# mbhall88/nohuman

Hardware: NVIDIA B200
Metric: classified+filtered throughput (Gbp/s) (higher is better)
Workload: dtype u64

## Files before the change

nohuman_b200/csrc/nh_kernels.cu:

```cuda
#include <stdlib.h>
#include <string.h>

#include "nh_kernels.cuh"

#define FULL_MASK 0xFFFFFFFFu


__device__ __forceinline__ uint32_t lane_id() { return threadIdx.x & 31u; }

__device__ __forceinline__ uint32_t warp_sum_u32(uint32_t v) {
  return __reduce_add_sync(FULL_MASK, v);
}

__device__ __forceinline__ uint64_t block_excl_scan(uint64_t v, uint64_t *total,
                                                    uint64_t *s_warp ) {
  uint32_t lane = lane_id(), warp = threadIdx.x >> 5;
  uint64_t inc = v;
#pragma unroll
  for (int d = 1; d < 32; d <<= 1) {
    uint64_t o = __shfl_up_sync(FULL_MASK, inc, d);
    if (lane >= (uint32_t)d) inc += o;
  }
  if (lane == 31) s_warp[warp] = inc;
  __syncthreads();
// ... 672 lines not shown
template <bool SMEM_PARENT>
__global__ void __launch_bounds__(NH_BLOCK_THREADS)
k_score(const NhDbParams db, const NhBatchPtrs b, const NhScoreParams sp) {
  extern __shared__ uint32_t s_dyn[];
  uint32_t *s_parent = s_dyn;
  const uint32_t parent_words = SMEM_PARENT ? db.node_count : 0u;
  uint32_t *s_hash = s_dyn + parent_words;
  if (SMEM_PARENT) {
    for (uint32_t i = threadIdx.x; i < db.node_count; i += blockDim.x) s_parent[i] = db.parent[i];
    __syncthreads();
  }
  const uint32_t *parent = SMEM_PARENT ? s_parent : db.parent;
  const uint32_t lane = lane_id(), warp = threadIdx.x >> 5;
  uint32_t *keys = s_hash + warp * 2u * NH_WARP_HASH_SLOTS;
  uint32_t *cnts = keys + NH_WARP_HASH_SLOTS;
  uint32_t classified = 0, kept = 0;
  const uint32_t wstride = gridDim.x * NH_WARPS_PER_BLOCK;
  const uint32_t n_todo = b.deferred_units ? b.counters->n_deferred : b.n_units;
  for (uint32_t i = blockIdx.x * NH_WARPS_PER_BLOCK + warp; i < n_todo; i += wstride) {
    const uint32_t u = b.deferred_units ? b.deferred_units[i] : i;
    acc_begin(keys, cnts, NH_WARP_HASH_SLOTS - 1u, lane);
    const UnitAcc a = b.tile_tab != nullptr ? acc_from_tile_tables(db, b, keys, cnts, NH_WARP_HASH_SLOTS - 1u, u, lane)
                                            : acc_from_lookups(db, b, keys, cnts, NH_WARP_HASH_SLOTS - 1u, u, lane);
    if (!resolve_unit(db, b, sp, parent, keys, cnts, NH_WARP_HASH_SLOTS - 1u, u, lane, a, &classified, &kept)) {
      if (lane == 0) b.overflow_units[atomicAdd(&b.counters->n_overflow, 1u)] = u;
    }
  }
  if (lane == 0) {
    if (classified) atomicAdd(&b.counters->n_classified, classified);
    if (kept) atomicAdd(&b.counters->n_kept, kept);
  }
}

__global__ void __launch_bounds__(32)
k_score_big(const NhDbParams db, const NhBatchPtrs b, const NhScoreParams sp) {
  extern __shared__ uint32_t s_dyn[];
  __shared__ MinWarpSmem s_min;
  uint32_t *keys = s_dyn;
  uint32_t *cnts = s_dyn + NH_BIG_HASH_SLOTS;
  const uint32_t lane = lane_id();
  const uint32_t n = b.counters->n_overflow;
  uint32_t classified = 0, kept = 0;
  for (uint32_t i = blockIdx.x; i < n; i += gridDim.x) {
    const uint32_t u = b.overflow_units[i];
    acc_begin(keys, cnts, NH_BIG_HASH_SLOTS - 1u, lane);
    const UnitAcc a = acc_rescan(db, b, keys, cnts, NH_BIG_HASH_SLOTS - 1u, u, lane, s_min);
    if (!resolve_unit(db, b, sp, db.parent, keys, cnts, NH_BIG_HASH_SLOTS - 1u, u, lane, a, &classified, &kept)) {
      if (db.huge_slots == 0u) {
        if (lane == 0) atomicExch(&b.counters->error, 1u);
        continue;
      }
      uint32_t *gkeys = db.huge_table, *gcnts = db.huge_table + db.huge_slots, *lock = db.huge_table + 2u * db.huge_slots;
      if (lane == 0)
        while (atomicCAS(lock, 0u, 1u) != 0u) __nanosleep(200);
      __syncwarp();
      __threadfence();
      acc_begin(gkeys, gcnts, db.huge_slots - 1u, lane);
      const UnitAcc ga = acc_rescan(db, b, gkeys, gcnts, db.huge_slots - 1u, u, lane, s_min);
      const bool ok = resolve_unit(db, b, sp, db.parent, gkeys, gcnts, db.huge_slots - 1u, u, lane, ga, &classified, &kept);
      __threadfence();
      __syncwarp();
      if (lane == 0) {
        atomicExch(lock, 0u);
        if (!ok) atomicExch(&b.counters->error, 1u);
      }
    }
  }
  if (lane == 0) {
    if (classified) atomicAdd(&b.counters->n_classified, classified);
    if (kept) atomicAdd(&b.counters->n_kept, kept);
  }
}


#ifndef NH_BCHUNK_WORDS
#define NH_BCHUNK_WORDS 8u
#endif
#define NH_BCHUNK_STRIDE (NH_BCHUNK_WORDS * 4u + 16u)
#ifndef NH_PQ_SLOTS
#define NH_PQ_SLOTS 128u
#endif
#define NH_META_FIRST 0x8000u
#define NH_AUX_NONE 0xFFFFFFFFu
#ifndef NH_FILTER_RECENT
#define NH_FILTER_RECENT 4u
#endif
#define NH_AUX_FILTER 0x80000000u

template <bool EMIT>
struct __align__(16) StreamWarpSmem {
  uint4 pq[NH_PQ_SLOTS];
  uint32_t q_unit[32];
  uint32_t q_ckey[32];
  uint32_t q_aux[32];
  uint64_t first_min[32], last_min[32];
  uint32_t keys[NH_LANE_TAXA * 32];
  uint32_t cnts[NH_LANE_TAXA * 32];
  uint32_t groups[32];
  uint8_t owner[32];
  uint32_t overflow;
  uint32_t first_hit;
  uint64_t bbar[2], sbar;
  __align__(16) uint8_t bchunk[2][32 * NH_BCHUNK_STRIDE];
  __align__(16) uint32_t sect[32 * 8];
  uint32_t q_slot[EMIT ? 32 : 1];
  uint8_t recent[32];
};

#ifndef NH_STREAM_MIN_BLOCKS
#define NH_STREAM_MIN_BLOCKS 3
#endif
static_assert((sizeof(StreamWarpSmem<false>) * NH_WARPS_PER_BLOCK + 1024 + 512) * NH_STREAM_MIN_BLOCKS <= 227 * 1024,
              "k_stream_classify would no longer fit its blocks per SM");

template <typename SM>
__device__ __forceinline__ uint32_t lane_tab_get(const SM &sm, uint32_t lane, uint32_t n, uint32_t taxon) {
  for (uint32_t i = 0; i < n; i++)
    if (sm.keys[i * 32u + lane] == taxon) return sm.cnts[i * 32u + lane];
  return 0;
}

__device__ __forceinline__ uint32_t smem_addr(const void *p) { return (uint32_t)__cvta_generic_to_shared(p); }
__device__ __forceinline__ void mbar_init(uint32_t bar, uint32_t count) {
  asm volatile("mbarrier.init.shared::cta.b64 [%0], %1;" ::"r"(bar), "r"(count) : "memory");
}
__device__ __forceinline__ void cp_async16(uint32_t dst, const void *src) {
  asm volatile("cp.async.cg.shared.global [%0], [%1], 16;" ::"r"(dst), "l"(src) : "memory");
}
__device__ __forceinline__ void cp_async8(uint32_t dst, const void *src) {
  asm volatile("cp.async.ca.shared.global [%0], [%1], 8;" ::"r"(dst), "l"(src) : "memory");
}
__device__ __forceinline__ void cp_async4(uint32_t dst, const void *src) {
  asm volatile("cp.async.ca.shared.global [%0], [%1], 4;" ::"r"(dst), "l"(src) : "memory");
}
__device__ __forceinline__ void cp_async16_zfill(uint32_t dst, const void *src, uint32_t n_src) {
  asm volatile("cp.async.cg.shared.global [%0], [%1], 16, %2;" ::"r"(dst), "l"(src), "r"(n_src) : "memory");
}
__device__ __forceinline__ void cp_async16_l2_64(uint32_t dst, const void *src) {
  asm volatile("cp.async.cg.shared.global.L2::64B [%0], [%1], 16;" ::"r"(dst), "l"(src) : "memory");
}
__device__ __forceinline__ void cp_async_arrive(uint32_t bar) {
  asm volatile("cp.async.mbarrier.arrive.noinc.shared::cta.b64 [%0];" ::"r"(bar) : "memory");
}
__device__ __forceinline__ void mbar_wait(uint32_t bar, uint32_t parity) {
  asm volatile(
      "{\n"
      ".reg .pred p;\n"
      "NH_WAIT:\n"
      "mbarrier.try_wait.parity.shared::cta.b64 p, [%0], %1;\n"
      "@p bra NH_DONE;\n"
      "bra NH_WAIT;\n"
      "NH_DONE:\n"
      "}" ::"r"(bar),
      "r"(parity)
      : "memory");
}
__device__ __forceinline__ uint32_t lds_u32(uint32_t addr) {
  uint32_t v;
  asm volatile("ld.shared.u32 %0, [%1];" : "=r"(v) : "r"(addr));
  return v;
}


__device__ __forceinline__ uint32_t nh_filter_hash(uint32_t ckey) {
  uint32_t h = ckey * 0x9E3779B1u;
  h ^= h >> 15;
  h *= 0x85EBCA77u;
  h ^= h >> 13;
  return h;
}

__global__ void __launch_bounds__(256)
k_filter_build(const uint32_t *__restrict__ cells, uint64_t capacity, uint32_t value_bits, uint32_t value_mask,
               uint32_t *__restrict__ filter, uint32_t n_blocks) {
  const uint32_t blk = blockIdx.x * blockDim.x + threadIdx.x;
  if (blk >= n_blocks) return;
  uint32_t rec[8];
#pragma unroll
  for (int i = 0; i < 8; i++) rec[i] = 0;
  const uint64_t base = (uint64_t)blk * 32ULL;
#pragma unroll 1
  for (uint32_t q = 0; q < 8; q++) {
    uint32_t c[4] = {0u, 0u, 0u, 0u};
    if (base + q * 4u + 4u <= capacity) {
      const uint4 v = __ldg(reinterpret_cast<const uint4 *>(cells + base) + q);
      c[0] = v.x; c[1] = v.y; c[2] = v.z; c[3] = v.w;
    } else {
      for (uint32_t j = 0; j < 4; j++)
        if (base + q * 4u + j < capacity) c[j] = __ldg(cells + base + q * 4u + j);
    }
#pragma unroll
    for (uint32_t j = 0; j < 4; j++) {
      const uint32_t cell = q * 4u + j;
      if (base + cell >= capacity) {
        rec[0] |= 1u << cell;
      } else if (c[j] & value_mask) {
        rec[0] |= 1u << cell;
        const uint32_t h = nh_filter_hash(c[j] >> value_bits);
        const uint32_t i0 = h & 63u, i1 = (h >> 6) & 63u, i2 = (h >> 12) & 63u, i3 = (h >> 18) & 31u;
        rec[1 + (i0 >> 5)] |= 1u << (i0 & 31u);
        rec[3 + (i1 >> 5)] |= 1u << (i1 & 31u);
        rec[5 + (i2 >> 5)] |= 1u << (i2 & 31u);
        rec[7] |= 1u << i3;
      }
    }
  }
  uint4 *out = reinterpret_cast<uint4 *>(filter + (uint64_t)blk * 8ULL);
  out[0] = make_uint4(rec[0], rec[1], rec[2], rec[3]);
  out[1] = make_uint4(rec[4], rec[5], rec[6], rec[7]);
}

#ifndef NH_STREAM_CHECK_MASK
#define NH_STREAM_CHECK_MASK 1
#endif

template <int W, int KL, bool DBG, bool REV0, bool EMIT, bool PACKED, int FILTER>
__global__ void __launch_bounds__(NH_BLOCK_THREADS, NH_STREAM_MIN_BLOCKS)
k_stream_classify(const NhDbParams db, const NhBatchPtrs b, const NhScoreParams sp) {
  static_assert(W == 5, "the scan consumes one 4-byte word per ring rotation");
  static_assert(NH_PQ_SLOTS >= 31u + 32u * (NH_STREAM_CHECK_MASK + 1u), "runs closed between two probe checks must fit the ring");
  static_assert((NH_PQ_SLOTS & (NH_PQ_SLOTS - 1u)) == 0 && (NH_BCHUNK_WORDS & (NH_BCHUNK_WORDS - 1u)) == 0, "powers of two");
  typedef StreamWarpSmem<EMIT> Smem;
  extern __shared__ __align__(16) uint32_t s_dyn[];
  uint32_t *s_parent = s_dyn;
  const bool smem_parent = db.node_count <= NH_SMEM_PARENT_MAX;
  const uint32_t parent_words = smem_parent ? db.node_count : 0u;
  Smem *s_warps = reinterpret_cast<Smem *>(s_dyn + ((parent_words + 3u) & ~3u));
  if (smem_parent) {
    for (uint32_t i = threadIdx.x; i < db.node_count; i += blockDim.x) s_parent[i] = db.parent[i];
    __syncthreads();
  }
  const uint32_t *parent = smem_parent ? s_parent : db.parent;
  const uint32_t lane = lane_id(), warp = threadIdx.x >> 5;
  const uint32_t lane_lt = (1u << lane) - 1u;
  Smem &sm = s_warps[warp];
  const uint32_t n_tiles = b.counters->n_tiles;
  const int k = KL ? 35 : db.k, l = KL ? 31 : db.l;
  const uint32_t amb_span = KL ? 34u : (uint32_t)db.amb_span;
  const uint64_t lmask = (1ULL << (2 * l)) - 1ULL;
  const uint32_t rc_shift = 2u * (uint32_t)(l - 1);
  const uint32_t n_sectors = (uint32_t)((db.capacity + 7ULL) >> 3);
  const uint32_t last_sector = n_sectors - 1u;
  const uint32_t last_range = (db.capacity & 7ULL) ? (1u << (uint32_t)(db.capacity & 7ULL)) - 1u : 0xFFu;
  const uint32_t max_visits = FILTER ? (n_sectors + 1u < 0x7FFEu ? n_sectors + 1u : 0x7FFEu) : (n_sectors + 1u < 0xFFFFu ? n_sectors + 1u : 0xFFFFu);
  const uint32_t last_block = FILTER ? sp.n_filter_blocks - 1u : 0u;
  const uint32_t ck_bits = 32u - db.value_bits;
  uint32_t tot_lookups = 0, tot_sectors = 0, tot_classified = 0, tot_kept = 0;

  const uint32_t bar0 = smem_addr(&sm.bbar[0]);
  const uint32_t win0 = smem_addr(&sm.bchunk[0][lane * NH_BCHUNK_STRIDE]);
  const uint32_t sbar = smem_addr(&sm.sbar);
  const uint32_t sect0 = smem_addr(&sm.sect[0]);
  uint32_t bar_par = 0;
  uint32_t sect_par = 0;
  if (lane == 0) {
    mbar_init(bar0, 32u);
    mbar_init(bar0 + 8u, 32u);
    mbar_init(sbar, 32u);
    asm volatile("fence.mbarrier_init.release.cluster;" ::: "memory");
  }
  asm volatile("fence.proxy.async.shared::cta;" ::: "memory");
  __syncwarp();

  for (;;) {
    uint32_t group = 0;
    if (lane == 0) group = atomicAdd(&b.counters->next_group, 1u);
    group = __shfl_sync(FULL_MASK, group, 0);
    if ((uint64_t)group * 32ULL >= n_tiles) break;
    const uint32_t tile = group * 32u + lane;
    const bool have = tile < n_tiles;
    NhTile t;
    t.seq = 0; t.pos_begin = 0; t.slot = 0; t.role = NH_ROLE_DEFERRED;
    if (have) t = b.tiles[tile];
    const uint32_t kind = NH_ROLE_KIND(t.role);
    const uint32_t owner = kind == NH_ROLE_MEMBER ? lane - NH_ROLE_DELTA(t.role) : lane;
#pragma unroll
    for (int i = 0; i < NH_LANE_TAXA; i++) {
      sm.keys[i * 32 + lane] = 0;
      sm.cnts[i * 32 + lane] = 0;
    }
    sm.groups[lane] = 0;
    if (FILTER == 3) sm.recent[lane] = 0;
    sm.owner[lane] = (uint8_t)owner;
    if (lane == 0) {
      sm.overflow = 0;
      sm.first_hit = 0;
    }
    __syncwarp();

    uint32_t pq_head = 0, pq_n = 0, cq_n = 0;
    uint32_t n_popped = 0;
    uint32_t n_conts = 0;
    uint32_t f_unit = 0, f_ckey = 0, f_slot = 0, f_aux = NH_AUX_NONE, f_start = 0;
    bool any_inflight = false;

    auto probe_round = [&]() {
      if (any_inflight) {
        const bool active = f_aux != NH_AUX_NONE;
        bool done = false;
        uint32_t result = 0;
        mbar_wait(sbar, sect_par);
        sect_par ^= 1u;
        if (active) {
          uint32_t c[8];
          {
            const uint4 lo = *reinterpret_cast<const uint4 *>(&sm.sect[lane * 8u]);
            const uint4 hi = *reinterpret_cast<const uint4 *>(&sm.sect[lane * 8u + 4u]);
            c[0] = lo.x; c[1] = lo.y; c[2] = lo.z; c[3] = lo.w;
            c[4] = hi.x; c[5] = hi.y; c[6] = hi.z; c[7] = hi.w;
          }
          if (FILTER) {
            const uint32_t ck = f_ckey & ((1u << ck_bits) - 1u);
            const uint32_t st = f_ckey >> ck_bits;
            const uint32_t visits = ((f_aux >> 16) & 0x7FFFu) + 1u;
            f_ckey = ck;
            if (f_aux & NH_AUX_FILTER) {
              const uint32_t h = nh_filter_hash(ck);
              const uint32_t w0 = (h & 32u) ? c[2] : c[1], w1 = (h & (32u << 6)) ? c[4] : c[3], w2 = (h & (32u << 12)) ? c[6] : c[5];
              const bool maybe = (((w0 >> (h & 31u)) & (w1 >> ((h >> 6) & 31u)) & (w2 >> ((h >> 12) & 31u)) & (c[7] >> ((h >> 18) & 31u))) & 1u) != 0u;
              const uint32_t free_cells = ~c[0] & (0xFFFFFFFFu << st);
              if (!maybe && free_cells != 0u) {
                done = true;
              } else if (visits >= max_visits) {
                done = true;
                atomicOr(&sm.overflow, FULL_MASK);
              } else if (maybe) {
                f_aux = (f_aux & 0xFFFFu) | (visits << 16);
                f_unit = f_unit * 4u + (st >> 3);
                f_ckey = ck | ((st & 7u) << ck_bits);
              } else {
                f_aux = (f_aux & (NH_AUX_FILTER | 0xFFFFu)) | (visits << 16);
                f_unit = f_unit == last_block ? 0u : f_unit + 1u;
              }
            } else {
              uint32_t range = 0xFFu << st;
              if (f_unit == last_sector) range &= last_range;
              int state = -1;
#pragma unroll
              for (int j = 7; j >= 0; j--) {
                const uint32_t val = c[j] & db.value_mask;
                const bool term = (val == 0u) || ((c[j] >> db.value_bits) == ck);
                if (term && ((range >> j) & 1u)) state = (int)val;
              }
              if (state >= 0) {
                done = true;
                result = (uint32_t)state;
              } else if (visits >= max_visits) {
                done = true;
                atomicOr(&sm.overflow, FULL_MASK);
              } else {
                f_aux = (f_aux & 0xFFFFu) | (visits << 16);
                f_unit = f_unit == last_sector ? 0u : f_unit + 1u;
              }
            }
          } else {
          uint32_t range = 0xFFu << f_start;
          if (f_unit == last_sector) range &= last_range;
          int state = -1;
#pragma unroll
          for (int j = 7; j >= 0; j--) {
            const uint32_t val = c[j] & db.value_mask;
            const bool term = (val == 0u) || ((c[j] >> db.value_bits) == f_ckey);
            if (term && ((range >> j) & 1u)) state = (int)val;
          }
          if (state >= 0) {
            done = true;
            result = (uint32_t)state;
          } else {
            const uint32_t visits = (f_aux >> 16) + 1u;
            if (visits >= max_visits) {
              done = true;
              if (EMIT) result = cht_walk(db, (uint64_t)f_unit * 8ULL + f_start, f_ckey);
              else atomicOr(&sm.overflow, FULL_MASK);
            } else {
              f_aux = (f_aux & 0xFFFFu) | (visits << 16);
              f_unit = f_unit == last_sector ? 0u : f_unit + 1u;
            }
          }
          }
        }
        const bool cont = active && !done;
        const uint32_t cmask = __ballot_sync(FULL_MASK, cont);
        if (cont) {
          const uint32_t pos = cq_n + __popc(cmask & lane_lt);
          sm.q_unit[pos] = f_unit;
          sm.q_ckey[pos] = f_ckey;
          sm.q_aux[pos] = f_aux;
          if (EMIT) sm.q_slot[pos] = f_slot;
        }
        cq_n += __popc(cmask);
        if (active && done) {
          const uint32_t tile_lane = f_aux & 31u;
          if (EMIT) b.lk_taxon[f_slot] = result;
          if (FILTER == 3) {
            const uint32_t r = sm.recent[tile_lane];
            if (result) sm.recent[tile_lane] = NH_FILTER_RECENT;
            else if (r) sm.recent[tile_lane] = (uint8_t)(r - 1u);
          }
          if (result) {
            const uint32_t own = sm.owner[tile_lane];
            const uint32_t n = (f_aux >> 5) & 0x3FFu;
            if (f_aux & NH_META_FIRST) atomicOr(&sm.first_hit, 1u << tile_lane);
            atomicAdd(&sm.groups[own], 1u);
            int i = 0;
            for (; i < sp.lane_taxa; i++) {
              const uint32_t old = atomicCAS(&sm.keys[i * 32 + own], 0u, result);
              if (old == 0u || old == result) {
                atomicAdd(&sm.cnts[i * 32 + own], n);
                break;
              }
            }
            if (i == sp.lane_taxa) atomicOr(&sm.overflow, 1u << own);
          }
        }
      }
      __syncwarp();
      const uint32_t n_cq = cq_n;
      const uint32_t room = 32u - n_cq;
      const uint32_t n_pq = pq_n < room ? pq_n : room;
      f_aux = NH_AUX_NONE;
      f_start = 0;
      if (lane < n_cq) {
        f_unit = sm.q_unit[lane];
        f_ckey = sm.q_ckey[lane];
        f_aux = sm.q_aux[lane];
        if (EMIT) f_slot = sm.q_slot[lane];
      } else if (lane - n_cq < n_pq) {
        const uint4 e = sm.pq[(pq_head + (lane - n_cq)) & (NH_PQ_SLOTS - 1u)];
        const uint64_t h = nh_fmix64(((uint64_t)e.y << 32) | e.x);
        if (EMIT) f_slot = e.w;
        const uint32_t meta = e.z;
        if (db.min_hash && h < db.min_hash) {
          if (EMIT) b.lk_taxon[f_slot] = 0u;
        } else {
          const uint64_t idx = nh_fastmod(h, db.capacity, db.mod_m, db.mod_sh1, db.mod_sh2);
          if (FILTER) {
            const bool ask = FILTER == 2 || (FILTER == 3 ? sm.recent[meta & 31u] == 0u : sm.groups[sm.owner[meta & 31u]] == 0u);
            const uint32_t st = (uint32_t)idx & (ask ? 31u : 7u);
            f_unit = (uint32_t)(idx >> (ask ? 5 : 3));
            f_ckey = (uint32_t)(h >> (32u + db.value_bits)) | (st << ck_bits);
            f_aux = ask ? (meta | NH_AUX_FILTER) : meta;
          } else {
            f_unit = (uint32_t)(idx >> 3);
            f_start = (uint32_t)idx & 7u;
            f_ckey = (uint32_t)(h >> (32u + db.value_bits));
            f_aux = meta;
          }
        }
      }
      cq_n = 0;
      pq_head = (pq_head + n_pq) & (NH_PQ_SLOTS - 1u);
      pq_n -= n_pq;
      n_popped += n_pq;
      n_conts += n_cq;
      any_inflight = (n_cq + n_pq) != 0u;
      if (any_inflight) {
        const uint32_t mine = f_aux != NH_AUX_NONE ? f_unit : 0xFFFFFFFFu;
        const uint32_t half = lane & 1u, src_lane = lane >> 1;
        const uint32_t u0 = __shfl_sync(FULL_MASK, mine, src_lane);
        const uint32_t u1 = __shfl_sync(FULL_MASK, mine, 16u + src_lane);
        const uint32_t dst = sect0 + src_lane * 32u + half * 16u;
        const uint32_t *src0 = db.cells, *src1 = db.cells;
        if (FILTER) {
          const uint32_t fmask = __ballot_sync(FULL_MASK, f_aux != NH_AUX_NONE && (f_aux & NH_AUX_FILTER));
          if ((fmask >> src_lane) & 1u) src0 = sp.filter;
          if ((fmask >> (16u + src_lane)) & 1u) src1 = sp.filter;
        }
        if (u0 != 0xFFFFFFFFu) cp_async16_l2_64(dst, src0 + (uint64_t)u0 * 8ULL + half * 4u);
        if (u1 != 0xFFFFFFFFu) cp_async16_l2_64(dst + 512u, src1 + (uint64_t)u1 * 8ULL + half * 4u);
        cp_async_arrive(sbar);
      }
      __syncwarp();
    };

    uint32_t n_runs = 0;
    uint32_t first_flag = NH_META_FIRST;
    uint64_t last = NH_NONE64;
    {
      uint64_t so = 0;
      uint32_t nb = 0;
      if (have) {
        so = b.offsets[t.seq];
        const uint32_t len = (uint32_t)(b.offsets[t.seq + 1] - so);
        uint32_t npos = len - (uint32_t)k + 1u - t.pos_begin;
        if (npos > (uint32_t)db.tile_pos) npos = (uint32_t)db.tile_pos;
        nb = npos + (uint32_t)k - 1u;
      }
      const uint8_t *g = PACKED ? nullptr : b.bases + so + t.pos_begin;
      const uint32_t mis = PACKED ? 0u : (uint32_t)((uintptr_t)g & 3u);
      const uint32_t my_words = have ? (mis + nb + 3u) >> 2 : 0u;
      const uint32_t max_words = __reduce_max_sync(FULL_MASK, my_words);

      uint64_t fwd = 0, rc = 0;
      uint64_t ring[4], pair[2];
#pragma unroll
      for (int i = 0; i < 4; i++) ring[i] = NH_NONE64;
      pair[0] = pair[1] = NH_NONE64;
      uint32_t c_run = 0;
      uint32_t cnt = 0;
      const uint64_t dbg_base = DBG && have ? b.dbg_pos_offsets[t.seq] + t.pos_begin : 0;
      const uint32_t first_pos = mis + (uint32_t)(k - 1);
      const uint32_t end_idx = mis + nb;

      auto emit = [&](bool pred, uint64_t key, uint32_t count) {
        const uint32_t emask = __ballot_sync(FULL_MASK, pred);
        if (pred) {
          uint4 e;
          e.x = (uint32_t)key;
          e.y = (uint32_t)(key >> 32);
          e.z = lane | (count << 5) | first_flag;
          e.w = 0;
          if (EMIT) {
            e.w = t.slot + n_runs;
            b.lk_cnt[e.w] = (uint16_t)count;
          }
          sm.pq[(pq_head + pq_n + __popc(emask & lane_lt)) & (NH_PQ_SLOTS - 1u)] = e;
          if (first_flag) sm.first_min[lane] = key;
          first_flag = 0;
          if (EMIT || DBG) n_runs++;
        }
        pq_n += __popc(emask);
      };

      auto scan_quad = [&](const uint32_t codes , const uint32_t ambs, const uint32_t base_i) {
#pragma unroll
        for (int j = 0; j < 4; j++) {
          const uint32_t i = base_i + (uint32_t)j;
          const uint32_t cc = (codes >> (6u - 2u * (uint32_t)j)) & 3u;
          const bool amb = (ambs >> j) & 1u;
          fwd = ((fwd << 2) | cc) & lmask;
          rc = (rc >> 2) | ((uint64_t)(3u - cc) << rc_shift);
          c_run = amb ? 0u : c_run + 1u;
          uint64_t cand = NH_NONE64;
          if (c_run >= (uint32_t)l) {
            const bool rev0 = REV0 || (DBG && db.revcom_version == 0);
            const uint64_t rcv = rev0 ? (((rc << (64 - 2 * l)) | ((1ULL << (64 - 2 * l)) - 1ULL)) & lmask) : rc;
            cand = ((fwd < rcv ? fwd : rcv) & db.seed_mask) ^ db.toggle;
          }
          const uint64_t a_i = min_u64(cand, ring[0]);
          const uint64_t m = min_u64(min_u64(a_i, pair[1]), ring[3]);
          pair[1] = pair[0];
          pair[0] = a_i;
#pragma unroll
          for (int r = 3; r > 0; r--) ring[r] = ring[r - 1];
          ring[0] = cand;
          const bool nonamb = i >= first_pos && c_run >= amb_span;
          const uint64_t mz = m ^ db.toggle;
          if (DBG && i >= first_pos && i < end_idx) {
            const uint64_t o = dbg_base + (i - first_pos);
            b.dbg_pos_min[o] = mz;
            b.dbg_pos_ambig[o] = nonamb ? 0 : 1;
          }
          const bool newrun = nonamb && mz != last;
          emit(newrun && cnt != 0u, last, cnt);
          cnt = newrun ? 1u : cnt + (nonamb ? 1u : 0u);
          last = newrun ? mz : last;
          if ((j & NH_STREAM_CHECK_MASK) == NH_STREAM_CHECK_MASK) {
            while (pq_n >= 32u) probe_round();
          }
        }
      };

      auto scan_word = [&](const uint32_t word, const uint32_t base_i) {
        uint32_t ambs;
        const uint32_t codes = nh_pack4(word, &ambs);
        scan_quad(codes, ambs, base_i);
      };

      if (PACKED) {
        const uint64_t unit0 = have ? (uint64_t)b.poff[t.seq] + (t.pos_begin >> 5) : 0ULL;
        const uint32_t my_units = have ? (nb + 31u) >> 5 : 0u;
        const uint32_t n_chunks = (max_words + 7u) >> 3;
        auto stage = [&](const uint32_t ch) {
          const uint32_t buf = ch & 1u;
          const uint32_t dst = win0 + buf * (32u * NH_BCHUNK_STRIDE);
          if (ch < my_units) {
            cp_async8(dst, b.codes + (unit0 + ch) * 8ULL);
            cp_async4(dst + 8u, b.valid + unit0 + ch);
          }
          cp_async_arrive(bar0 + buf * 8u);
        };
        if (n_chunks) stage(0u);
        for (uint32_t ch = 0; ch < n_chunks; ch++) {
          if (ch + 1u < n_chunks) stage(ch + 1u);
          const uint32_t buf = ch & 1u;
          mbar_wait(bar0 + buf * 8u, (bar_par >> buf) & 1u);
          bar_par ^= 1u << buf;
          const uint32_t wbase = win0 + buf * (32u * NH_BCHUNK_STRIDE);
          const uint32_t c_lo = lds_u32(wbase), c_hi = lds_u32(wbase + 4u);
          uint32_t vw = lds_u32(wbase + 8u);
          const int rem = (int)nb - (int)(ch * 32u);
          vw = rem <= 0 ? 0u : (rem >= 32 ? vw : vw & ((1u << rem) - 1u));
          const uint32_t amb_w = ~vw;
          const uint32_t q0 = ch * 8u;
          const uint32_t qn = max_words - q0 < 8u ? max_words - q0 : 8u;
#pragma unroll 1
          for (uint32_t qd = 0; qd < qn; qd++) {
            const uint32_t cw = qd < 4u ? c_lo : c_hi;
            scan_quad((cw >> ((qd & 3u) * 8u)) & 0xFFu, (amb_w >> (qd * 4u)) & 0xFu, (q0 + qd) * 4u);
          }
          __syncwarp();
        }
        emit(cnt != 0u, last, cnt);
      } else {
      const uint8_t *q = g - mis;
      const uint32_t a16 = (uint32_t)((uintptr_t)q & 15u);
      const uint8_t *src0 = q - a16;
      const uint32_t my_bytes = have ? a16 + mis + nb : 0u;
      const uint32_t n_chunks = (max_words + NH_BCHUNK_WORDS - 1u) / NH_BCHUNK_WORDS;
      auto stage = [&](const uint32_t ch) {
        const uint32_t buf = ch & 1u;
        const uint32_t lo = ch * (NH_BCHUNK_WORDS * 4u);
        const uint32_t dst = win0 + buf * (32u * NH_BCHUNK_STRIDE);
#pragma unroll
        for (uint32_t pc = 0; pc < NH_BCHUNK_STRIDE; pc += 16u) {
          const uint32_t at = lo + pc;
          const uint32_t n_src = at < my_bytes ? (my_bytes - at < 16u ? my_bytes - at : 16u) : 0u;
          cp_async16_zfill(dst + pc, n_src ? src0 + at : src0, n_src);
        }
        cp_async_arrive(bar0 + buf * 8u);
      };
      if (n_chunks) stage(0u);
      for (uint32_t ch = 0; ch < n_chunks; ch++) {
        if (ch + 1u < n_chunks) stage(ch + 1u);
        const uint32_t buf = ch & 1u;
        mbar_wait(bar0 + buf * 8u, (bar_par >> buf) & 1u);
        bar_par ^= 1u << buf;
        const uint32_t wbase = win0 + buf * (32u * NH_BCHUNK_STRIDE) + a16;
        const uint32_t w0 = ch * NH_BCHUNK_WORDS;
        const uint32_t wn = max_words - w0 < NH_BCHUNK_WORDS ? max_words - w0 : NH_BCHUNK_WORDS;
        uint32_t w_next = lds_u32(wbase);
        if (ch == 0u) w_next &= 0xFFFFFFFFu << (8u * mis);
#pragma unroll 1
        for (uint32_t w = 0; w < wn; w++) {
          const uint32_t word = w_next;
          w_next = lds_u32(wbase + (((w + 1u) & (NH_BCHUNK_WORDS - 1u)) << 2));
          scan_word(word, (w0 + w) * 4u);
        }
        __syncwarp();
      }
      emit(cnt != 0u, last, cnt);
      }
    }
    const bool has_runs = first_flag == 0u;
    if (EMIT && have) {
      NhTileOut o;
      o.lk_off = t.slot;
      o.lk_cnt = n_runs;
      b.tile_out[tile] = o;
    }
    if (has_runs) sm.last_min[lane] = last;
    while (pq_n + cq_n != 0u || any_inflight) probe_round();
    tot_lookups += n_popped;
    tot_sectors += n_popped + n_conts;

    {
      __syncwarp();
      const uint32_t has_mask = __ballot_sync(FULL_MASK, has_runs);
      if (have && kind != NH_ROLE_DEFERRED && t.pos_begin != 0u && has_runs && ((sm.first_hit >> lane) & 1u)) {
        const uint32_t seq_lane = lane - t.pos_begin / (uint32_t)db.tile_pos;
        const uint32_t cand = has_mask & lane_lt & ~((1u << seq_lane) - 1u);
        if (cand) {
          const uint32_t pl = 31u - (uint32_t)__clz(cand);
          if (sm.last_min[pl] == sm.first_min[lane]) atomicSub(&sm.groups[owner], 1u);
        }
      }
      __syncwarp();
    }

    if (have && kind == NH_ROLE_DEFERRED) {
      const bool ovf = (sm.overflow >> lane) & 1u;
      NhTileSum ts;
      ts.first_min = has_runs ? sm.first_min[lane] : NH_NONE64;
      ts.last_min = has_runs ? last : NH_NONE64;
      ts.groups = sm.groups[lane];
      ts.flags = (has_runs ? NH_TILE_HAS : 0u) | (((sm.first_hit >> lane) & 1u) ? NH_TILE_FIRST_HIT : 0u) |
                 (ovf ? NH_TILE_OVERFLOW : 0u);
      b.tile_sum[tile] = ts;
      if (!ovf) {
        NhTileTab tt;
#pragma unroll
        for (int i = 0; i < NH_LANE_TAXA; i++) {
          tt.keys[i] = sm.keys[i * 32 + lane];
          tt.cnts[i] = sm.cnts[i * 32 + lane];
        }
        b.tile_tab[tile] = tt;
      }
    }

    if (have && kind == NH_ROLE_LEADER) {
      const uint32_t u = b.paired ? (t.seq >> 1) : t.seq;
      if ((sm.overflow >> lane) & 1u) {
        b.overflow_units[atomicAdd(&b.counters->n_overflow, 1u)] = u;
      } else {
        uint32_t ntab = 0;
        while (ntab < (uint32_t)sp.lane_taxa && sm.keys[ntab * 32u + lane] != 0u) ntab++;
        const int groups = (int)sm.groups[lane];
        const uint32_t total_kmers = unit_total_kmers(db, b, u);
        uint32_t best_s = 0, best_t = 0;
        for (uint32_t i = 0; i < ntab; i++) {
          const uint32_t tx = sm.keys[i * 32u + lane];
          uint32_t score = 0;
          for (uint32_t a = tx; a; a = parent[a]) score += lane_tab_get(sm, lane, ntab, a);
          if (score > best_s) {
            best_s = score;
            best_t = tx;
          } else if (score == best_s) {
            best_t = lca(parent, best_t, tx);
          }
        }
        uint32_t max_taxon = best_t;
        uint32_t max_score = max_taxon ? lane_tab_get(sm, lane, ntab, max_taxon) : 0u;
        const uint32_t required = (uint32_t)ceil(__dmul_rn(sp.confidence, (double)total_kmers));
        while (max_taxon && max_score < required) {
          uint32_t sum = 0;
          for (uint32_t i = 0; i < ntab; i++)
            if (is_a_ancestor_of_b(parent, max_taxon, sm.keys[i * 32u + lane]))
              sum += sm.cnts[i * 32u + lane];
          max_score = sum;
          if (max_score >= required) break;
          max_taxon = parent[max_taxon];
        }
        uint32_t call = max_taxon;
        if (call && groups < sp.min_hit_groups) call = 0;
        const uint32_t is_cls = call != 0u;
        const uint32_t keep = sp.keep_human ? is_cls : !is_cls;
        if (b.out_call) b.out_call[u] = call ? db.ext_id[call] : 0u;
        if (b.out_keep) b.out_keep[u] = (uint8_t)keep;
        if (b.dbg_call) b.dbg_call[u] = call;
        if (b.dbg_total_kmers) b.dbg_total_kmers[u] = total_kmers;
        if (b.dbg_hit_groups) b.dbg_hit_groups[u] = (uint32_t)groups;
        tot_classified += is_cls;
        tot_kept += keep;
      }
    }
    __syncwarp();
  }
  tot_classified = warp_sum_u32(tot_classified);
  tot_kept = warp_sum_u32(tot_kept);
  if (lane == 0) {
    if (tot_lookups) atomicAdd(&b.counters->n_lookups, tot_lookups);
    if (tot_sectors) atomicAdd(&b.counters->n_sector_reads, tot_sectors);
    if (tot_classified) atomicAdd(&b.counters->n_classified, tot_classified);
    if (tot_kept) atomicAdd(&b.counters->n_kept, tot_kept);
  }
}


__global__ void __launch_bounds__(NH_BLOCK_THREADS)
k_gather_runs(const NhDbParams db, const NhBatchPtrs b, uint32_t *__restrict__ run_ext,
              uint16_t *__restrict__ run_len, uint32_t *__restrict__ tile_run_off,
              uint32_t *__restrict__ cursor) {
  const uint32_t lane = lane_id(), warp = threadIdx.x >> 5;
  const uint32_t n_tiles = b.counters->n_tiles;
  for (uint32_t tile = blockIdx.x * NH_WARPS_PER_BLOCK + warp; tile < n_tiles;
       tile += gridDim.x * NH_WARPS_PER_BLOCK) {
    const NhTileOut to = b.tile_out[tile];
    uint32_t base = 0;
    if (lane == 0) base = to.lk_cnt ? atomicAdd(cursor, to.lk_cnt) : 0u;
    base = __shfl_sync(FULL_MASK, base, 0);
    if (lane == 0) tile_run_off[tile] = base;
    for (uint32_t j = lane; j < to.lk_cnt; j += 32u) {
      run_ext[base + j] = db.ext_id[b.lk_taxon[to.lk_off + j]];
      run_len[base + j] = b.lk_cnt[to.lk_off + j];
    }
  }
}

__device__ __forceinline__ void fetch_sector_async(const uint32_t *cells, uint64_t sector, uint32_t smem_slot0, uint32_t lane) {
  const uint32_t half = lane & 1u, src_lane = lane >> 1;
  const uint64_t u0 = __shfl_sync(FULL_MASK, sector, src_lane);
  const uint64_t u1 = __shfl_sync(FULL_MASK, sector, 16u + src_lane);
  const uint32_t dst = smem_slot0 + src_lane * 32u + half * 16u;
  cp_async16_l2_64(dst, cells + u0 * 8ULL + half * 4u);
  cp_async16_l2_64(dst + 512u, cells + u1 * 8ULL + half * 4u);
}

template <int DEPTH>
__global__ void __launch_bounds__(256)
k_probe_pattern_async(const uint32_t *__restrict__ cells, uint64_t n_sectors, uint32_t items_per_chain,
                      uint32_t p_thresh, uint64_t seed, unsigned long long *__restrict__ counters,
                      uint32_t *__restrict__ sink) {
  __shared__ __align__(16) uint32_t s_sect[8][DEPTH][32 * 8];
  const uint32_t lane = lane_id(), warp = threadIdx.x >> 5;
  const uint64_t chain0 = ((uint64_t)blockIdx.x * blockDim.x + threadIdx.x) * DEPTH;
  uint64_t blk[DEPTH];
  uint32_t left[DEPTH], cont[DEPTH];
  uint32_t acc = 0;
  unsigned long long items = 0, requests = 0;
#pragma unroll
  for (int d = 0; d < DEPTH; d++) {
    blk[d] = __umul64hi(nh_fmix64(seed + (chain0 + d) * 0x9E3779B97F4A7C15ULL), n_sectors);
    left[d] = items_per_chain;
    cont[d] = 0;
    fetch_sector_async(cells, blk[d], smem_addr(&s_sect[warp][d][0]), lane);
    asm volatile("cp.async.commit_group;" ::: "memory");
  }
  for (uint32_t it = 1; it <= 2u * items_per_chain + 2u; it++) {
#pragma unroll
    for (int d = 0; d < DEPTH; d++) {
      asm volatile("cp.async.wait_group %0;" ::"n"(DEPTH - 1) : "memory");
      __syncwarp();
      const uint4 lo = *reinterpret_cast<const uint4 *>(&s_sect[warp][d][lane * 8u]);
      const uint4 hi = *reinterpret_cast<const uint4 *>(&s_sect[warp][d][lane * 8u + 4u]);
      const uint32_t x = lo.x ^ lo.y ^ lo.z ^ lo.w ^ hi.x ^ hi.y ^ hi.z ^ hi.w;
      __syncwarp();
      if (left[d] != 0u) {
        acc ^= x;
        requests++;
        const uint64_t h = nh_fmix64(seed ^ ((chain0 + d) << 20) ^ it ^ (uint64_t)(x & 1u) << 63);
        if (!cont[d] && (uint32_t)h < p_thresh) {
          cont[d] = 1;
          blk[d] = blk[d] + 1 < n_sectors ? blk[d] + 1 : 0;
        } else {
          cont[d] = 0;
          items++;
          left[d]--;
          blk[d] = __umul64hi(h, n_sectors);
        }
      }
      fetch_sector_async(cells, blk[d], smem_addr(&s_sect[warp][d][0]), lane);
      asm volatile("cp.async.commit_group;" ::: "memory");
    }
    if (!__any_sync(FULL_MASK, left[0] != 0u || left[DEPTH - 1] != 0u)) break;
  }
  asm volatile("cp.async.wait_group 0;" ::: "memory");
  if (acc == 0x9E3779B9u) sink[0] = acc;
  items = __reduce_add_sync(FULL_MASK, (uint32_t)items);
  requests = __reduce_add_sync(FULL_MASK, (uint32_t)requests);
  if (lane == 0) {
    atomicAdd(&counters[0], items);
    atomicAdd(&counters[1], requests);
  }
}

template <int G, int DEPTH>
__global__ void __launch_bounds__(256)
k_probe_pattern(const uint32_t *__restrict__ cells, uint64_t n_sectors, uint32_t items_per_chain,
                uint32_t p_thresh , uint64_t seed, uint64_t sm_window_sectors,
                unsigned long long *__restrict__ counters , uint32_t *__restrict__ sink) {
  const uint32_t lane = lane_id();
  const uint32_t sub = lane % G;
  const uint64_t chain0 = (((uint64_t)blockIdx.x * blockDim.x + threadIdx.x) / G) * DEPTH;
  uint64_t win_base = 0, win_size = n_sectors / G;
  if (sm_window_sectors) {
    uint32_t smid;
    asm("mov.u32 %0, %%smid;" : "=r"(smid));
    win_size = sm_window_sectors / G;
    const uint64_t n_win = (n_sectors / G) / win_size;
    win_base = (uint64_t)(smid % (uint32_t)(n_win ? n_win : 1)) * win_size;
  }
  uint32_t acc = 0;
  uint32_t c[DEPTH][8];
  uint64_t blk[DEPTH];
  uint32_t left[DEPTH];
  uint32_t cont[DEPTH];
  unsigned long long items = 0, requests = 0;
#pragma unroll
  for (int d = 0; d < DEPTH; d++) {
    const uint64_t h = nh_fmix64(seed + (chain0 + d) * 0x9E3779B97F4A7C15ULL);
    blk[d] = win_base + __umul64hi(h, win_size);
    left[d] = items_per_chain;
    cont[d] = 0;
    ld_sector(cells + (blk[d] * G + sub) * 8ULL, c[d]);
  }
  bool busy = true;
  for (uint32_t it = 1; busy; it++) {
    busy = false;
#pragma unroll
    for (int d = 0; d < DEPTH; d++) {
      if (left[d] == 0u) continue;
      busy = true;
      const uint32_t x = c[d][0] ^ c[d][1] ^ c[d][2] ^ c[d][3] ^ c[d][4] ^ c[d][5] ^ c[d][6] ^ c[d][7];
      acc ^= x;
      requests++;
      const uint64_t h = nh_fmix64(seed ^ ((chain0 + d) << 20) ^ it ^ (uint64_t)(x & 1u) << 63);
      if (!cont[d] && (uint32_t)h < p_thresh) {
        cont[d] = 1;
        blk[d] = blk[d] + 1 < win_base + win_size ? blk[d] + 1 : win_base;
      } else {
        cont[d] = 0;
        items++;
        if (--left[d] == 0u) continue;
        blk[d] = win_base + __umul64hi(h, win_size);
      }
      ld_sector(cells + (blk[d] * G + sub) * 8ULL, c[d]);
    }
  }
  if (acc == 0x9E3779B9u) sink[0] = acc;
  if (sub == 0) {
    items = __reduce_add_sync(__activemask(), (uint32_t)items);
    requests = __reduce_add_sync(__activemask(), (uint32_t)requests);
    if (lane == 0) {
      atomicAdd(&counters[0], items);
      atomicAdd(&counters[1], requests);
    }
  }
}


template <bool EMIT>
static size_t stream_smem_bytes(uint32_t node_count) {
  const uint32_t parent_words = node_count <= NH_SMEM_PARENT_MAX ? node_count : 0u;
  return (size_t)((parent_words + 3u) & ~3u) * 4 + NH_WARPS_PER_BLOCK * sizeof(StreamWarpSmem<EMIT>);
}

cudaError_t nh_kernels_init(void) {
  cudaError_t e = cudaFuncSetAttribute(k_score_big, cudaFuncAttributeMaxDynamicSharedMemorySize,
                                       NH_BIG_HASH_SLOTS * 8);
  if (e != cudaSuccess) return e;
  e = cudaFuncSetAttribute(k_score<true>, cudaFuncAttributeMaxDynamicSharedMemorySize,
                           NH_SMEM_PARENT_MAX * 4 + NH_WARPS_PER_BLOCK * NH_WARP_HASH_SLOTS * 8);
  if (e != cudaSuccess) return e;
  const int smax = (int)stream_smem_bytes<false>(NH_SMEM_PARENT_MAX), smax_emit = (int)stream_smem_bytes<true>(NH_SMEM_PARENT_MAX);
#define NH_SET_SMEM(kern, bytes)                                                             \
  e = cudaFuncSetAttribute(kern, cudaFuncAttributeMaxDynamicSharedMemorySize, bytes);       \
  if (e != cudaSuccess) return e;
  NH_SET_SMEM((k_stream_classify<5, 1, false, false, false, false, 0>), smax)
  NH_SET_SMEM((k_stream_classify<5, 1, false, false, true, false, 0>), smax_emit)
  NH_SET_SMEM((k_stream_classify<5, 0, false, false, false, false, 0>), smax)
  NH_SET_SMEM((k_stream_classify<5, 0, false, true, false, false, 0>), smax)
  NH_SET_SMEM((k_stream_classify<5, 0, true, false, false, false, 0>), smax)
  NH_SET_SMEM((k_stream_classify<5, 0, false, false, true, false, 0>), smax_emit)
  NH_SET_SMEM((k_stream_classify<5, 0, false, true, true, false, 0>), smax_emit)
  NH_SET_SMEM((k_stream_classify<5, 1, false, false, false, true, 0>), smax)
  NH_SET_SMEM((k_stream_classify<5, 0, false, false, false, true, 0>), smax)
  NH_SET_SMEM((k_stream_classify<5, 0, false, true, false, true, 0>), smax)
  NH_SET_SMEM((k_stream_classify<5, 1, false, false, false, false, 1>), smax)
  NH_SET_SMEM((k_stream_classify<5, 1, false, false, false, false, 2>), smax)
  NH_SET_SMEM((k_stream_classify<5, 1, false, false, false, false, 3>), smax)
  NH_SET_SMEM((k_stream_classify<5, 1, false, false, false, true, 1>), smax)
  NH_SET_SMEM((k_stream_classify<5, 1, false, false, false, true, 2>), smax)
  NH_SET_SMEM((k_stream_classify<5, 1, false, false, false, true, 3>), smax)
#undef NH_SET_SMEM
  return cudaSuccess;
}

void nh_launch_filter_build(const NhDbParams &db, uint32_t *filter, uint32_t n_blocks, cudaStream_t st) {
  k_filter_build<<<(n_blocks + 255u) / 256u, 256, 0, st>>>(db.cells, db.capacity, db.value_bits, db.value_mask, filter, n_blocks);
}

int nh_launch_len_scan(const uint32_t *len, uint32_t n_seqs, uint64_t *sums, uint64_t *off, uint32_t *poff, cudaStream_t st) {
  const uint32_t nb = (n_seqs + PLAN_THREADS - 1) / PLAN_THREADS;
  if (nb == 0) return 0;
  k_len_count<<<nb, PLAN_THREADS, 0, st>>>(len, n_seqs, sums);
  k_len_scan<<<1, PLAN_THREADS, 0, st>>>(sums, nb);
  k_len_fill<<<nb, PLAN_THREADS, 0, st>>>(len, n_seqs, sums, off, poff);
  return 3;
}

int nh_launch_plan(const NhDbParams &db, const NhBatchPtrs &b, cudaStream_t st) {
  const uint32_t nb = (b.n_seqs + PLAN_THREADS - 1) / PLAN_THREADS;
  k_plan_count<<<nb, PLAN_THREADS, 0, st>>>(b.offsets, b.n_seqs, db.k, db.tile_pos, b.block_sums);
  k_plan_scan<<<1, PLAN_THREADS, 0, st>>>(b.block_sums, nb, b.counters);
  k_plan_fill<<<nb, PLAN_THREADS, 0, st>>>(b.offsets, b.n_seqs, db.k, db.tile_pos, b.paired,
                                           b.deferred_units != nullptr, b.block_sums, b.tile_base,
                                           b.tiles, b.deferred_units, b.counters, b.seq_info);
  if (b.seq_info == nullptr) return 3;
  uint32_t blocks = (b.tiles_upper + 255u) / 256u;
  if (blocks > 148u * 16u) blocks = 148u * 16u;
  k_plan_tiles<<<blocks ? blocks : 1u, 256, 0, st>>>(b.tile_base, b.seq_info, b.n_seqs, db.tile_pos, b.tiles, b.counters);
  return 4;
}

bool nh_fused_supported(const NhDbParams &db) {
  return db.w == 5 && db.tile_pos <= NH_FUSED_TILE_POS_MAX && db.capacity < (1ULL << 35) - 8ULL;
}

int nh_launch_stream(const NhDbParams &db, const NhBatchPtrs &b, const NhScoreParams &sp,
                     uint32_t tiles_upper, int sm_count, cudaStream_t st) {
  const uint32_t groups = (tiles_upper + 31u) / 32u;
  const uint32_t blocks = (groups + NH_WARPS_PER_BLOCK - 1) / NH_WARPS_PER_BLOCK;
  const uint32_t smax = (uint32_t)sm_count * NH_STREAM_MIN_BLOCKS;
  uint32_t grid = blocks < smax ? blocks : smax;
  if (grid == 0) grid = 1;
  const bool emit = b.emit_all_taxa != 0;
  const size_t smem = emit ? stream_smem_bytes<true>(db.node_count) : stream_smem_bytes<false>(db.node_count);
// ... 107 lines not shown
```

Measured before the change: 117.7.

## Unify probe termination logic, add first-slot taxon fast path, defer toggle XOR

Result: faster. 120.0, median of 6 (+1.9%).

```diff
diff --git a/nohuman_b200/csrc/nh_kernels.cu b/nohuman_b200/csrc/nh_kernels.cu
--- a/nohuman_b200/csrc/nh_kernels.cu
+++ b/nohuman_b200/csrc/nh_kernels.cu
@@ -998,81 +998,45 @@
         mbar_wait(sbar, sect_par);
         sect_par ^= 1u;
         if (active) {
-          uint32_t c[8];
-          {
-            const uint4 lo = *reinterpret_cast<const uint4 *>(&sm.sect[lane * 8u]);
-            const uint4 hi = *reinterpret_cast<const uint4 *>(&sm.sect[lane * 8u + 4u]);
-            c[0] = lo.x; c[1] = lo.y; c[2] = lo.z; c[3] = lo.w;
-            c[4] = hi.x; c[5] = hi.y; c[6] = hi.z; c[7] = hi.w;
+          const uint4 lo = *reinterpret_cast<const uint4 *>(&sm.sect[lane * 8u]);
+          const uint4 hi = *reinterpret_cast<const uint4 *>(&sm.sect[lane * 8u + 4u]);
+          const uint32_t c[8] = {lo.x, lo.y, lo.z, lo.w, hi.x, hi.y, hi.z, hi.w};
+          const uint32_t ck = FILTER ? f_ckey & ((1u << ck_bits) - 1u) : f_ckey;
+          const uint32_t st = FILTER ? f_ckey >> ck_bits : f_start;
+          const uint32_t visits = FILTER ? ((f_aux >> 16) & 0x7FFFu) + 1u : (f_aux >> 16) + 1u;
+          const bool is_filter = FILTER && (f_aux & NH_AUX_FILTER);
+          bool maybe = false;
+          uint32_t fin;
+          if (is_filter) {
+            const uint32_t h = nh_filter_hash(ck);
+            const uint32_t w0 = (h & 32u) ? c[2] : c[1], w1 = (h & (32u << 6)) ? c[4] : c[3], w2 = (h & (32u << 12)) ? c[6] : c[5];
+            maybe = (((w0 >> (h & 31u)) & (w1 >> ((h >> 6) & 31u)) & (w2 >> ((h >> 12) & 31u)) & (c[7] >> ((h >> 18) & 31u))) & 1u) != 0u;
+            fin = maybe ? 0u : ~c[0] & (0xFFFFFFFFu << st);
+          } else {
+            fin = 0u;
+#pragma unroll
+            for (int j = 0; j < 8; j++)
+              fin |= (uint32_t)(((c[j] & db.value_mask) == 0u) | ((c[j] >> db.value_bits) == ck)) << j;
+            uint32_t range = 0xFFu << st;
+            if (f_unit == last_sector) range &= last_range;
+            fin &= range;
           }
-          if (FILTER) {
-            const uint32_t ck = f_ckey & ((1u << ck_bits) - 1u);
-            const uint32_t st = f_ckey >> ck_bits;
-            const uint32_t visits = ((f_aux >> 16) & 0x7FFFu) + 1u;
+          if (fin != 0u) {
+            done = true;
+            if (!is_filter) result = lds_u32(sect0 + (lane * 8u + (uint32_t)(__ffs(fin) - 1)) * 4u) & db.value_mask;
+          } else if (visits >= max_visits) {
+            done = true;
+            if (EMIT) result = cht_walk(db, (uint64_t)f_unit * 8ULL + st, ck);
+            else atomicOr(&sm.overflow, FULL_MASK);
+          } else if (maybe) {
+            f_aux = (f_aux & 0xFFFFu) | (visits << 16);
+            f_unit = f_unit * 4u + (st >> 3);
+            f_ckey = ck | ((st & 7u) << ck_bits);
+          } else {
+            f_aux = (f_aux & (FILTER ? NH_AUX_FILTER | 0xFFFFu : 0xFFFFu)) | (visits << 16);
+            const uint32_t last_unit = is_filter ? last_block : last_sector;
+            f_unit = f_unit == last_unit ? 0u : f_unit + 1u;
             f_ckey = ck;
-            if (f_aux & NH_AUX_FILTER) {
-              const uint32_t h = nh_filter_hash(ck);
-              const uint32_t w0 = (h & 32u) ? c[2] : c[1], w1 = (h & (32u << 6)) ? c[4] : c[3], w2 = (h & (32u << 12)) ? c[6] : c[5];
-              const bool maybe = (((w0 >> (h & 31u)) & (w1 >> ((h >> 6) & 31u)) & (w2 >> ((h >> 12) & 31u)) & (c[7] >> ((h >> 18) & 31u))) & 1u) != 0u;
-              const uint32_t free_cells = ~c[0] & (0xFFFFFFFFu << st);
-              if (!maybe && free_cells != 0u) {
-                done = true;
-              } else if (visits >= max_visits) {
-                done = true;
-                atomicOr(&sm.overflow, FULL_MASK);
-              } else if (maybe) {
-                f_aux = (f_aux & 0xFFFFu) | (visits << 16);
-                f_unit = f_unit * 4u + (st >> 3);
-                f_ckey = ck | ((st & 7u) << ck_bits);
-              } else {
-                f_aux = (f_aux & (NH_AUX_FILTER | 0xFFFFu)) | (visits << 16);
-                f_unit = f_unit == last_block ? 0u : f_unit + 1u;
-              }
-            } else {
-              uint32_t range = 0xFFu << st;
-              if (f_unit == last_sector) range &= last_range;
-              int state = -1;
-#pragma unroll
-              for (int j = 7; j >= 0; j--) {
-                const uint32_t val = c[j] & db.value_mask;
-                const bool term = (val == 0u) || ((c[j] >> db.value_bits) == ck);
-                if (term && ((range >> j) & 1u)) state = (int)val;
-              }
-              if (state >= 0) {
-                done = true;
-                result = (uint32_t)state;
-              } else if (visits >= max_visits) {
-                done = true;
-                atomicOr(&sm.overflow, FULL_MASK);
-              } else {
-                f_aux = (f_aux & 0xFFFFu) | (visits << 16);
-                f_unit = f_unit == last_sector ? 0u : f_unit + 1u;
-              }
-            }
-          } else {
-          uint32_t range = 0xFFu << f_start;
-          if (f_unit == last_sector) range &= last_range;
-          int state = -1;
-#pragma unroll
-          for (int j = 7; j >= 0; j--) {
-            const uint32_t val = c[j] & db.value_mask;
-            const bool term = (val == 0u) || ((c[j] >> db.value_bits) == f_ckey);
-            if (term && ((range >> j) & 1u)) state = (int)val;
-          }
-          if (state >= 0) {
-            done = true;
-            result = (uint32_t)state;
-          } else {
-            const uint32_t visits = (f_aux >> 16) + 1u;
-            if (visits >= max_visits) {
-              done = true;
-              if (EMIT) result = cht_walk(db, (uint64_t)f_unit * 8ULL + f_start, f_ckey);
-              else atomicOr(&sm.overflow, FULL_MASK);
-            } else {
-              f_aux = (f_aux & 0xFFFFu) | (visits << 16);
-              f_unit = f_unit == last_sector ? 0u : f_unit + 1u;
-            }
-          }
           }
         }
         const bool cont = active && !done;
@@ -1099,7 +1063,8 @@
             if (f_aux & NH_META_FIRST) atomicOr(&sm.first_hit, 1u << tile_lane);
             atomicAdd(&sm.groups[own], 1u);
             int i = 0;
-            for (; i < sp.lane_taxa; i++) {
+            if (sm.keys[own] == result) atomicAdd(&sm.cnts[own], n);
+            else for (; i < sp.lane_taxa; i++) {
               const uint32_t old = atomicCAS(&sm.keys[i * 32 + own], 0u, result);
               if (old == 0u || old == result) {
                 atomicAdd(&sm.cnts[i * 32 + own], n);
@@ -1123,7 +1088,7 @@
         if (EMIT) f_slot = sm.q_slot[lane];
       } else if (lane - n_cq < n_pq) {
         const uint4 e = sm.pq[(pq_head + (lane - n_cq)) & (NH_PQ_SLOTS - 1u)];
-        const uint64_t h = nh_fmix64(((uint64_t)e.y << 32) | e.x);
+        const uint64_t h = nh_fmix64((((uint64_t)e.y << 32) | e.x) ^ db.toggle);
         if (EMIT) f_slot = e.w;
         const uint32_t meta = e.z;
         if (db.min_hash && h < db.min_hash) {
@@ -1241,16 +1206,15 @@
           for (int r = 3; r > 0; r--) ring[r] = ring[r - 1];
           ring[0] = cand;
           const bool nonamb = i >= first_pos && c_run >= amb_span;
-          const uint64_t mz = m ^ db.toggle;
           if (DBG && i >= first_pos && i < end_idx) {
             const uint64_t o = dbg_base + (i - first_pos);
-            b.dbg_pos_min[o] = mz;
+            b.dbg_pos_min[o] = m ^ db.toggle;
             b.dbg_pos_ambig[o] = nonamb ? 0 : 1;
           }
-          const bool newrun = nonamb && mz != last;
+          const bool newrun = nonamb && m != last;
           emit(newrun && cnt != 0u, last, cnt);
           cnt = newrun ? 1u : cnt + (nonamb ? 1u : 0u);
-          last = newrun ? mz : last;
+          last = newrun ? m : last;
           if ((j & NH_STREAM_CHECK_MASK) == NH_STREAM_CHECK_MASK) {
             while (pq_n >= 32u) probe_round();
           }
@@ -1367,8 +1331,8 @@
     if (have && kind == NH_ROLE_DEFERRED) {
       const bool ovf = (sm.overflow >> lane) & 1u;
       NhTileSum ts;
-      ts.first_min = has_runs ? sm.first_min[lane] : NH_NONE64;
-      ts.last_min = has_runs ? last : NH_NONE64;
+      ts.first_min = has_runs ? sm.first_min[lane] ^ db.toggle : NH_NONE64;
+      ts.last_min = has_runs ? last ^ db.toggle : NH_NONE64;
       ts.groups = sm.groups[lane];
       ts.flags = (has_runs ? NH_TILE_HAS : 0u) | (((sm.first_hit >> lane) & 1u) ? NH_TILE_FIRST_HIT : 0u) |
                  (ovf ? NH_TILE_OVERFLOW : 0u);
```
